# meco-group/omg-tools

Measured on AMD Instinct MI355X. Metric: MPC solves/sec, 1024-agent Holonomic Point2point batch per GPU, higher is better.
Workload: dtype f64

## Files before the change

### omg-tools_amd/csrc/omgx_core.h

```cpp
#pragma once
#include <stdint.h>
#include <math.h>

#ifdef OMGX_HOST_PORT
#define OMGX_FN inline
#define OMGX_HD inline
#define OMGX_HDF inline
#else
#define OMGX_FN __device__ __forceinline__
#define OMGX_HD __host__ __device__ inline
#define OMGX_HDF __host__ __device__ __forceinline__
#endif

#ifdef OMGX_HOST_PORT
#include <vector>
static thread_local std::vector<double> omgx_rbak;
#endif
#ifdef OMGX_COUNT_FACT
#include <atomic>
static std::atomic<long> omgx_dbg_nfact(0);
static std::atomic<long> omgx_dbg_cnt[12];
#endif
namespace omgx {

// ... 839 lines not shown
  const bool is_row = c.tid() < total_rows;
  const bool is_blk = wave >= row_waves && wave < row_waves + nm;
  int r = c.tid();
  BMat M = Ms[0];
  if (is_row) { int mi = 0; while (r >= Ms[mi].rows) { r -= Ms[mi].rows; ++mi; } M = Ms[mi]; }
  else if (is_blk) { M = Ms[wave - row_waves]; r = -1; }
  double* iv = (M.dinv >= 0) ? dinvb + M.dinv : colb + M.pan;
  double* gb = colb + M.pan + M.nfact;
  double* bb = gb + 16;
  const int br = baddr_k<KIND>(M, r > 0 ? r : 0, 0);
  int badl = 0;
  for (int jb = 0; jb < nmax; jb += OMGX_NB) {
    const bool live = (is_row || is_blk) && jb < M.nfact;
    const int nb = (M.nfact - jb) < OMGX_NB ? (M.nfact - jb) : OMGX_NB;
    const int q1 = nb > 1 ? 1 : 0, q2 = nb > 2 ? 2 : 0, q3 = nb > 3 ? 3 : 0;
    double v0 = 0.0, v1 = 0.0, v2 = 0.0, v3 = 0.0;
    if (live && is_blk) {
      const int a = lane & 15, kq = lane >> 4;
      const bool in_blk = a < nb;
      const int ra = baddr_k<KIND>(M, jb + (in_blk ? a : 0), 0);
      typedef double v4d __attribute__((ext_vector_type(4)));
      v4d acc = {0.0, 0.0, 0.0, 0.0}, acc2 = {0.0, 0.0, 0.0, 0.0};
      int k0 = 0;
      for (; k0 + 8 <= jb; k0 += 8) {
        const double u_a = A[ra + k0 + kq], t_a = iv[k0 + kq], u_b = A[ra + k0 + 4 + kq], t_b = iv[k0 + 4 + kq];
        const double ua = in_blk ? u_a : 0.0, ub = in_blk ? u_b : 0.0;
        acc = __builtin_amdgcn_mfma_f64_16x16x4f64(ua * t_a, ua, acc, 0, 0, 0);
        acc2 = __builtin_amdgcn_mfma_f64_16x16x4f64(ub * t_b, ub, acc2, 0, 0, 0);
      }
      for (; k0 < jb; k0 += 4) {
        const double u_a = A[ra + k0 + kq], t_a = iv[k0 + kq];
        const double ua = in_blk ? u_a : 0.0;
        acc = __builtin_amdgcn_mfma_f64_16x16x4f64(ua * t_a, ua, acc, 0, 0, 0);
      }
      acc += acc2;
      {
        const int gr = lane >> 4, gc = lane & 15;
        if (gc <= gr) {
          const bool ok = gr < nb && gc < nb;
          const double orig = A[baddr_k<KIND>(M, jb + (ok ? gr : 0), jb + (ok ? gc : 0))];
          gb[gr * 4 + gc] = ok ? orig - acc[0] : (gr == gc ? 1.0 : 0.0);
        }
      }
      c.wave_sync();
      const Blk4 B = blk4_from(gb[0], gb[4], gb[5], gb[8], gb[9], gb[10], gb[12], gb[13], gb[14], gb[15]);
      if (lane == 0) {
        bb[0] = B.l10; bb[1] = B.l20; bb[2] = B.l21; bb[3] = B.l30; bb[4] = B.l31; bb[5] = B.l32;
        bb[6] = B.d0; bb[7] = B.d1; bb[8] = B.d2; bb[9] = B.d3;
      }
      if (lane < nb) {
        const double dq = lane == 0 ? B.d0 : (lane == 1 ? B.d1 : (lane == 2 ? B.d2 : B.d3));
        const double iq = lane == 0 ? B.i0 : (lane == 1 ? B.i1 : (lane == 2 ? B.i2 : B.i3));
        const bool pos_ok = (jb + lane < M.npos) ? (dq > 0.0) : (dq < 0.0);
        if (!pos_ok) badl = 1;
        bb[10 + lane] = iq;
      }
    } else if (live && r >= jb + nb) {
      const int b0 = baddr_k<KIND>(M, jb, 0), b1 = baddr_k<KIND>(M, jb + q1, 0), b2 = baddr_k<KIND>(M, jb + q2, 0), b3 = baddr_k<KIND>(M, jb + q3, 0);
      v0 = A[br + jb]; v1 = A[br + jb + q1]; v2 = A[br + jb + q2]; v3 = A[br + jb + q3];
#pragma unroll 4
      for (int k = 0; k < jb; ++k) {
        const double tk = iv[k], ur = A[br + k];
        const double w = ur * tk;
        v0 -= w * A[b0 + k]; v1 -= w * A[b1 + k]; v2 -= w * A[b2 + k]; v3 -= w * A[b3 + k];
      }
    }
    c.sync();
    if (live && is_row && r >= jb) {
      const double l10 = bb[0], l20 = bb[1], l21 = bb[2], l30 = bb[3], l31 = bb[4], l32 = bb[5];
      const double d0 = bb[6], d1 = bb[7], d2 = bb[8], d3 = bb[9];
      if (r < jb + nb) {
        const int q = r - jb;
        iv[jb + q] = bb[10 + q];
        if (q == 1) { A[br + jb] = l10 * d0; }
        else if (q == 2) { A[br + jb] = l20 * d0; A[br + jb + 1] = l21 * d1; }
        else if (q == 3) { A[br + jb] = l30 * d0; A[br + jb + 1] = l31 * d1; A[br + jb + 2] = l32 * d2; }
        A[br + jb + q] = q == 0 ? d0 : (q == 1 ? d1 : (q == 2 ? d2 : d3));
      } else {
        const double u0 = v0;
        const double u1 = v1 - u0 * l10;
        const double u2 = v2 - u0 * l20 - u1 * l21;
        const double u3 = v3 - u0 * l30 - u1 * l31 - u2 * l32;
        A[br + jb] = u0;
        if (nb > 1) A[br + jb + 1] = u1;
        if (nb > 2) A[br + jb + 2] = u2;
        if (nb > 3) A[br + jb + 3] = u3;
      }
    }
    c.sync();
  }
  *bad = c.rmax(badl ? 1.0 : 0.0) > 0.0 ? 1 : 0;
}
#endif

template <int KIND, class C>
OMGX_FN void ldl_blocked(const C& c, const BMat* Ms, int nm, double* A, double* dinvb, double* colb, double* stage, int* bad) {
  int nmax = 0, total_rows = 0;
  for (int i = 0; i < nm; ++i) { if (Ms[i].nfact > nmax) nmax = Ms[i].nfact; total_rows += Ms[i].rows; }
  int badl = 0;
  int mi_own = 0, r_own = c.tid();
  BMat M_own = Ms[0];
  if (c.tid() < total_rows) {
    while (r_own >= Ms[mi_own].rows) { r_own -= Ms[mi_own].rows; ++mi_own; }
    M_own = Ms[mi_own];
  }
  OMGX_TIC();
  for (int jb = 0; jb < nmax; jb += OMGX_NB) {
    OMGX_PFOR(it, total_rows) {
      int mi = mi_own, r = r_own;
      BMat M = M_own;
      if (it != c.tid()) {
        mi = 0; r = it;
        while (r >= Ms[mi].rows) { r -= Ms[mi].rows; ++mi; }
        M = Ms[mi];
      }
      if (jb >= M.nfact || r < jb) continue;
      const int nb = (M.nfact - jb) < OMGX_NB ? (M.nfact - jb) : OMGX_NB;
      const Blk4 B = blk4_factor<KIND>(M, A, jb, nb);
      if (r < jb + nb) {
        const int q = r - jb;
        double* st = stage + mi * OMGX_STAGE_LD + q * 4;
        const double dq = q == 0 ? B.d0 : (q == 1 ? B.d1 : (q == 2 ? B.d2 : B.d3));
        const double iq = q == 0 ? B.i0 : (q == 1 ? B.i1 : (q == 2 ? B.i2 : B.i3));
        if (q == 1) { st[0] = B.l10; }
        else if (q == 2) { st[0] = B.l20; st[1] = B.l21; }
        else if (q == 3) { st[0] = B.l30; st[1] = B.l31; st[2] = B.l32; }
        st[q] = dq;
        const bool pos_ok = (jb + q < M.npos) ? (dq > 0.0) : (dq < 0.0);
        if (!pos_ok) badl = 1;
        if (M.dinv >= 0) dinvb[M.dinv + jb + q] = iq;
        stage[mi * OMGX_STAGE_LD + 16 + q] = iq;
        if (q == 0) for (int qq = nb; qq < OMGX_NB; ++qq) stage[mi * OMGX_STAGE_LD + 16 + qq] = 0.0;
        double* pr = colb + M.pan + r * OMGX_PAN_LD;
        pr[0] = 0.0; pr[1] = 0.0; pr[2] = 0.0; pr[3] = 0.0;
      } else {
        const int base = baddr_k<KIND>(M, r, jb);
        const double a0 = A[base];
        const double l1 = A[base + (nb > 1 ? 1 : 0)], l2 = A[base + (nb > 2 ? 2 : 0)], l3 = A[base + (nb > 3 ? 3 : 0)];
        const double a1 = nb > 1 ? l1 : 0.0;
        const double a2 = nb > 2 ? l2 : 0.0;
        const double a3 = nb > 3 ? l3 : 0.0;
        const double u0 = a0;
        const double u1 = a1 - u0 * B.l10;
        const double u2 = a2 - u0 * B.l20 - u1 * B.l21;
        const double u3 = a3 - u0 * B.l30 - u1 * B.l31 - u2 * B.l32;
        const double p0 = u0 * B.i0, p1 = nb > 1 ? u1 * B.i1 : 0.0, p2 = nb > 2 ? u2 * B.i2 : 0.0,
                     p3 = nb > 3 ? u3 * B.i3 : 0.0;
        double* pr = colb + M.pan + r * OMGX_PAN_LD;
        pr[0] = u0; pr[1] = nb > 1 ? u1 : 0.0; pr[2] = nb > 2 ? u2 : 0.0; pr[3] = nb > 3 ? u3 : 0.0;
        const bool fact_row = r < M.nfact;
        A[base] = fact_row ? p0 : u0;
        if (nb > 1) A[base + 1] = fact_row ? p1 : u1;
        if (nb > 2) A[base + 2] = fact_row ? p2 : u2;
        if (nb > 3) A[base + 3] = fact_row ? p3 : u3;
      }
    }
    c.sync();
    OMGX_TOC(PH_LA);
    OMGX_PFOR(it, nm * 16) {
      const int mi = it >> 4, q = (it >> 2) & 3, k = it & 3;
      const BMat M = Ms[mi];
      if (jb < M.nfact && jb + q < M.nfact && k <= q) A[baddr_k<KIND>(M, jb + q, jb + k)] = stage[mi * OMGX_STAGE_LD + (it & 15)];
    }
    OMGX_TOC(PH_LS);
    int tile0 = 0;
    for (int mi = 0; mi < nm; ++mi) {
      const BMat M = Ms[mi];
      const int s0 = jb + OMGX_NB;
      if (s0 >= M.nfact) continue;
      const int tr = (M.rows - s0 + 15) >> 4, tc = (M.nfact - s0 + 15) >> 4;
#ifdef OMGX_HOST_PORT
      (void)tile0; (void)tr; (void)tc;
      for (int r = s0; r < M.rows; ++r) {
        const int kmax = r < M.nfact ? r : M.nfact - 1;
        for (int k = s0; k <= kmax; ++k) {
          double acc = 0.0;
          for (int q = 0; q < OMGX_NB; ++q)
            acc += colb[M.pan + r * OMGX_PAN_LD + q] * (colb[M.pan + k * OMGX_PAN_LD + q] * stage[mi * OMGX_STAGE_LD + 16 + q]);
          A[baddr_k<KIND>(M, r, k)] -= acc;
        }
      }
#else
      const int lane = c.lane(), nwm = c.nwaves() - 1;
      for (int ti = (c.wave() - tile0) & nwm; ti < tr; ti += nwm + 1) {
        const int R0 = s0 + 16 * ti;
        for (int tj = 0; tj < tc; ++tj) {
          const int K0 = s0 + 16 * tj;
          if (K0 > R0 + 15 && R0 + 15 < M.nfact) break;
          const int ra = R0 + (lane & 15), kb = K0 + (lane & 15), q = lane >> 4;
          const double av_l = colb[M.pan + (ra < M.rows ? ra : M.rows - 1) * OMGX_PAN_LD + q];
          const double bv_l = colb[M.pan + (kb < M.nfact ? kb : M.nfact - 1) * OMGX_PAN_LD + q];
          const double iv_l = stage[mi * OMGX_STAGE_LD + 16 + q];
          typedef double v4d __attribute__((ext_vector_type(4)));
          v4d acc;
          const int col = K0 + (lane & 15);
          int ad[4]; bool ok[4];
#pragma unroll
          for (int i = 0; i < 4; ++i) {
            const int row = R0 + (lane >> 4) + 4 * i;
            ok[i] = row < M.rows && col < M.nfact && (row >= M.nfact || col <= row);
            ad[i] = ok[i] ? baddr_k<KIND>(M, row, col) : M.a;
          }
          double al[4];
#pragma unroll
          for (int i = 0; i < 4; ++i) al[i] = A[ad[i]];
#pragma unroll
          for (int i = 0; i < 4; ++i) acc[i] = ok[i] ? al[i] : 0.0;
          const double av = (ra < M.rows) ? -av_l : 0.0;
          const double bv = (kb < M.nfact) ? bv_l * iv_l : 0.0;
          acc = __builtin_amdgcn_mfma_f64_16x16x4f64(av, bv, acc, 0, 0, 0);
#pragma unroll
          for (int i = 0; i < 4; ++i) if (ok[i]) A[ad[i]] = acc[i];
        }
      }
      tile0 += tr;
#endif
    }
    c.sync();
    OMGX_TOC(PH_LB);
  }
  *bad = c.rmax(badl ? 1.0 : 0.0) > 0.0 ? 1 : 0;
}

template <bool WAVE_ONLY, bool HBM, bool ROOT_LDS>
OMGX_HDF void kkt_describe_fill(const Dims& d, const Kkt& K, BMat* Ms) {
  const int pan0 = (OMGX_BMAT_DOUBLES + OMGX_STAGE_LD) * (OMGX_MAX_LEAF + 1);
  int pan = pan0;
  for (int l = 0; l < d.n_leaf; ++l) {
    BMat& M = Ms[l];
    if constexpr (WAVE_ONLY) {
      M.a = K.d_off[l]; M.ld = K.ld(l); M.nfact = K.nl(l); M.rows = K.nl(l) + K.nc(l) + 1; M.npos = M.nfact;
      M.dinv = K.leaf_off[l]; M.pan = K.lf_w[l]; M.cpl = K.cpl_ptr[l]; M.bw = K.lf_kind[l] ? -1 : K.lf_band[l]; M.pad_ = K.lf_ldb[l];
      continue;
    }
    M.a = K.d_off[l]; M.ld = K.ld(l); M.nfact = K.nl(l); M.rows = K.nl(l) + K.nc(l) + 1; M.npos = M.nfact;
    M.dinv = K.leaf_off[l]; M.pan = pan; pan += HBM ? OMGX_PAN_SMALL(M.nfact) : OMGX_PAN_LD * M.rows; M.cpl = K.cpl_ptr[l]; M.bw = K.leaf_bw[l];
  }
  BMat& Mr = Ms[d.n_leaf];
  Mr.a = ROOT_LDS ? 0 : K.d_off[d.n_leaf]; Mr.ld = 0; Mr.nfact = d.nr; Mr.rows = d.nr + 1; Mr.npos = d.n_root; Mr.dinv = -1; Mr.pan = pan0; Mr.cpl = 0; Mr.bw = d.nr;
  Mr.pad_ = K.d_off[d.n_leaf];
}

template <class C>
OMGX_FN void kkt_describe(const C& c, const Dims& d, const Kkt& K, Work& w, bool sync_after = true) {
  const int who = c.nthr() > 64 ? 64 : 0;
  if (c.tid() == who) kkt_describe_fill<C::wave_only, C::hbm, C::root_lds>(d, K, (BMat*)w.col);
  if (sync_after) c.sync();
}

template <class C>
OMGX_FN void kkt_descriptors(const C& c, const Dims& d, const Tables& T, Work& w, bool sync_after = true) {
  if constexpr (C::wave_only) {
    const int t0 = c.nthr() > 64 ? 64 : 0, nt = c.nthr() > 64 ? 64 : c.nthr();
    const int i0 = c.tid() - t0, n = (d.n_leaf + 1) * (int)(sizeof(BMat) / sizeof(int32_t));
    int32_t* Ms = (int32_t*)w.col;
    if (i0 >= 0 && i0 < nt) for (int i = i0; i < n; i += nt) Ms[i] = T.bmat_img[i];
    if (sync_after) c.sync();
  } else {
    Kkt K; K.bind(d, T, w.kkt);
    kkt_describe(c, d, K, w, sync_after);
  }
}

#ifndef OMGX_HOST_PORT
OMGX_FN WPanel wpanel_leaf(const BMat& M) {
  WPanel P; P.base = M.a; P.ld = M.ld; P.n = M.nfact; P.nreg = M.rows - 2; P.nvec = 2; P.npos = M.nfact; P.bw = M.bw;
  P.vrow = M.rows - 2; P.band = M.bw; P.ldb = M.pad_; P.wbase = M.pan;
  return P;
}
OMGX_FN WPanel wpanel_root(const BMat& M, int n_root) {
  WPanel P; P.base = M.a; P.ld = 0; P.n = M.nfact; P.nreg = M.nfact; P.nvec = 1; P.npos = n_root; P.bw = M.nfact;
  P.vrow = M.nfact; P.band = -1; P.ldb = 0; P.wbase = 0;
  return P;
}

struct DiagLeaf { int base, n, S, dinv, dl; };
OMGX_FN DiagLeaf diag_leaf(const BMat& M) {
  DiagLeaf L;
  L.base = __builtin_amdgcn_readfirstlane(M.a); L.n = __builtin_amdgcn_readfirstlane(M.nfact);
  L.S = __builtin_amdgcn_readfirstlane(M.pan); L.dinv = __builtin_amdgcn_readfirstlane(M.dinv); L.dl = 4 * L.dinv;
  return L;
}

template <class C>
OMGX_FN int kkt_factor_wave(const C& c, const Dims& d, const Kkt& K, Work& w) {
  typedef double v4d __attribute__((ext_vector_type(4)));
  const BMat* Ms = (const BMat*)w.col;
  const int lane = c.lane(), wave = c.wave(), nw = c.nwaves();
  const int koff = (int)(w.kkt - omgx_lds);
  OMGX_TIC();
  int badl = 0;
#ifdef OMGX_PROFILE
  const long long tw0_ = clock64();
#endif
  for (int l = wave; l < d.n_leaf; l += nw) {
    const int kind_bw = __builtin_amdgcn_readfirstlane(Ms[l].bw);
    if (kind_bw < 0) {
      const DiagLeaf L = diag_leaf(Ms[l]);
      const double dj = w.kkt[L.base + (lane < L.n ? lane : 0)];
      if (lane < L.n) { w.dinv[L.dinv + lane] = rcp_pivot(dj); if (!(dj > 0.0)) badl = 1; }
      continue;
    }
    const WPanel P = wpanel_leaf(Ms[l]);
    badl |= (kind_bw <= 8) ? wave_ldl<OMGX_WAVE_COLS, 8, true>(koff, P) : wave_ldl<OMGX_WAVE_COLS, OMGX_WAVE_COLS, true>(koff, P);
    wave_fence();
    const double dl = wave_dinv<true>(w.kkt, P);
    if (lane < P.n) w.dinv[Ms[l].dinv + lane] = dl;
  }
#ifdef OMGX_PROFILE
  if (c.tid() == 0) { c.prof[PH_F_SCALE] += clock64() - tw0_; c.prof[PH_F_PARK] += 1; }
#endif
  if (c.rmax(badl ? 1.0 : 0.0) > 0.0) return 1;
  OMGX_TOC(PH_F_LEAF);
  double* R = K.R();
  for (int base = 0; base < d.n_leaf; base += nw) {
    const int l = base + wave;
    v4d acc00 = {0.0, 0.0, 0.0, 0.0}, acc10 = acc00, acc11 = acc00;
    int nc1 = 0, ci_b0 = 0, ci_b1 = 0, ci_a[8];
    bool sparse = false;
#pragma unroll
    for (int i = 0; i < 8; ++i) ci_a[i] = 0;
    if (l < d.n_leaf) {
      const BMat M = Ms[l];
      sparse = __builtin_amdgcn_readfirstlane(M.bw) < 0;
      if (!sparse) {
      const int n = __builtin_amdgcn_readfirstlane(M.nfact), ld = __builtin_amdgcn_readfirstlane(M.ld);
      nc1 = __builtin_amdgcn_readfirstlane(M.rows) - n;
      const double* Wt = w.kkt + __builtin_amdgcn_readfirstlane(M.pan);
      const double* di = w.dinv + __builtin_amdgcn_readfirstlane(M.dinv);
      const int32_t* ci = K.cpl_idx + __builtin_amdgcn_readfirstlane(M.cpl);
      const int cb0 = lane & 15, cb1 = 16 + (lane & 15);
      ci_b0 = ci[cb0 < nc1 - 1 ? cb0 : 0]; ci_b1 = ci[cb1 < nc1 - 1 ? cb1 : 0];
#pragma unroll
      for (int i = 0; i < 8; ++i) {
        const int ca = 16 * (i >> 2) + (lane >> 4) + 4 * (i & 3);
        ci_a[i] = ca < nc1 - 1 ? ci[ca] : d.nr;
      }
      const int r0 = lane & 15, r1 = 16 + (lane & 15), q = lane >> 4;
      const int r0c = r0 < nc1 ? r0 : nc1 - 1, r1c = r1 < nc1 ? r1 : nc1 - 1;
      const bool two = nc1 > 16;
      for (int j0 = 0; j0 < n; j0 += 4) {
        const int j = j0 + q, jc = j < n ? j : n - 1;
        const double w0 = Wt[r0c * ld + jc], w1 = Wt[r1c * ld + jc], dj = di[jc];
        const double b0 = (r0 < nc1 && j < n) ? w0 : 0.0, b1 = (r1 < nc1 && j < n) ? w1 : 0.0;
        acc00 = __builtin_amdgcn_mfma_f64_16x16x4f64(b0 * dj, b0, acc00, 0, 0, 0);
        if (two) {
          acc10 = __builtin_amdgcn_mfma_f64_16x16x4f64(b1 * dj, b0, acc10, 0, 0, 0);
          acc11 = __builtin_amdgcn_mfma_f64_16x16x4f64(b1 * dj, b1, acc11, 0, 0, 0);
        }
      }
      }
    }
    const int lend = base + nw < d.n_leaf ? base + nw : d.n_leaf;
    for (int lr = base; lr < lend; ++lr) {
      if (l == lr && !sparse) {
        const int cb0 = lane & 15, cb1 = 16 + (lane & 15);
#pragma unroll
        for (int i = 0; i < 4; ++i) {
          const int ca0 = (lane >> 4) + 4 * i, ca1 = 16 + ca0;
          if (ca0 < nc1 && cb0 < nc1 - 1 && cb0 <= ca0) R[tri(ci_a[i], ci_b0)] -= acc00[i];
          if (ca1 < nc1 && cb0 < nc1 - 1) R[tri(ci_a[4 + i], ci_b0)] -= acc10[i];
          if (ca1 < nc1 && cb1 < nc1 - 1 && cb1 <= ca1) R[tri(ci_a[4 + i], ci_b1)] -= acc11[i];
        }
      } else if (l == lr) {
        const DiagLeaf L = diag_leaf(Ms[l]);
        const int j = lane < L.n ? lane : 0;
        const bool on = lane < L.n;
        const double* A = w.kkt + L.base + j;
        const double di = w.dinv[L.dinv + j];
        const double vt = A[(1 + L.S) * L.n], rj = A[(2 + L.S) * L.n];
        const int pt = d.n_root - 1;
        double vs[4]; int ps[4];
#pragma unroll
        for (int s = 0; s < 4; ++s) {
          const bool has = s < L.S;
          ps[s] = has ? K.dl_pos[L.dl + s * L.n + j] : -1;
          const double v = A[(1 + (has ? s : 0)) * L.n];
          vs[s] = (has && on && ps[s] >= 0) ? v : 0.0;
        }
        if (on) {
#pragma unroll
          for (int s = 0; s < 4; ++s) {
            if (ps[s] < 0 || s >= L.S) continue;
            const double u = vs[s] * di;
#pragma unroll
            for (int s2 = 0; s2 <= s; ++s2) {
              if (ps[s2] < 0) continue;
              const int pa = ps[s] > ps[s2] ? ps[s] : ps[s2], pb = ps[s] > ps[s2] ? ps[s2] : ps[s];
              R[tri(pa, pb)] -= u * vs[s2];
            }
            R[tri(pt, ps[s])] -= u * vt;
            R[tri(d.nr, ps[s])] -= u * rj;
          }
        }
        const double stt = c.wave_sum(on ? vt * di * vt : 0.0), srt = c.wave_sum(on ? rj * di * vt : 0.0);
        if (lane == 0) { R[tri(pt, pt)] -= stt; R[tri(d.nr, pt)] -= srt; }
      }
      c.sync();
    }
  }
  OMGX_TOC(PH_F_SCHUR);
  int badr = 0;
  if (wave == 0) {
    const WPanel P = wpanel_root(Ms[d.n_leaf], d.n_root);
#ifdef OMGX_PROFILE
    const long long tr0_ = clock64();
#endif
    badr = wave_ldl<OMGX_WAVE_COLS, OMGX_WAVE_COLS, false>(koff, P);
#ifdef OMGX_PROFILE
    if (c.tid() == 0) c.prof[PH_F_SWEEP] += clock64() - tr0_;
#endif
  }
  const int bad = c.rmax(badr ? 1.0 : 0.0) > 0.0 ? 2 : 0;
  OMGX_TOC(PH_F_ROOT);
  return bad;
}

template <class C>
OMGX_FN int kkt_refactor_root_wave(const C& c, const Dims& d, const Kkt& K, Work& w) {
  const BMat* Ms = (const BMat*)w.col;
  const int koff = (int)(w.kkt - omgx_lds);
  OMGX_TIC();
  int badr = 0;
  if (c.wave() == 0) badr = wave_ldl<OMGX_WAVE_COLS, OMGX_WAVE_COLS, false>(koff, wpanel_root(Ms[d.n_leaf], d.n_root));
  const int bad = c.rmax(badr ? 1.0 : 0.0) > 0.0 ? 2 : 0;
  OMGX_TOC(PH_F_ROOT);
  return bad;
}

template <class C>
OMGX_FN void kkt_solve_wave(const C& c, const Dims& d, const Kkt& K, Work& w, double* sol) {
  const BMat* Ms = (const BMat*)w.col;
  const int lane = c.lane(), wave = c.wave(), nw = c.nwaves();
  const int koff = (int)(w.kkt - omgx_lds);
  OMGX_TIC();
  if (wave == 0) {
    const WPanel P = wpanel_root(Ms[d.n_leaf], d.n_root);
    const double dl = wave_dinv<false>(w.kkt, P);
    const double y = w.kkt[wcarried<false>(P, P.n) + (lane < P.n ? lane : 0)];
    const double x = wave_bwd<OMGX_WAVE_COLS, false>(koff, P, dl, y * dl);
    if (lane < P.n) sol[d.root_off + lane] = x;
  }
  c.sync();
  OMGX_TOC(PH_K_ROOT);
  double* xg = w.col + OMGX_BMAT_DOUBLES * (OMGX_MAX_LEAF + 1) + wave * 64;
  for (int l = wave; l < d.n_leaf; l += nw) {
    const BMat M = Ms[l];
    if (__builtin_amdgcn_readfirstlane(M.bw) < 0) {
      const DiagLeaf L = diag_leaf(M);
      const int j = lane < L.n ? lane : 0;
      const double* A = w.kkt + L.base + j;
      double acc = A[(2 + L.S) * L.n] - A[(1 + L.S) * L.n] * sol[d.root_off + d.n_root - 1];
      for (int s = 0; s < L.S; ++s) {
        const int ps = K.dl_pos[L.dl + s * L.n + j];
        acc = fma(-A[(1 + s) * L.n], sol[d.root_off + (ps < 0 ? 0 : ps)] * (ps < 0 ? 0.0 : 1.0), acc);
      }
      if (lane < L.n) sol[L.dinv + lane] = acc * w.dinv[L.dinv + j];
      continue;
    }
    const WPanel P = wpanel_uniform(wpanel_leaf(M));
    const int n = P.n, nc = P.nreg + 1 - P.n, ld = P.ld;
    const int32_t* ci = K.cpl_idx + __builtin_amdgcn_readfirstlane(M.cpl);
    if (lane < nc) xg[lane] = sol[d.root_off + ci[lane]];
    wave_fence();
    const int j = lane < n ? lane : 0;
    const double* Wt = w.kkt + P.wbase + j;
    double acc = Wt[nc * ld];
#pragma unroll 4
    for (int a = 0; a < nc; ++a) acc = fma(-Wt[a * ld], xg[a], acc);
    const int dv = __builtin_amdgcn_readfirstlane(M.dinv);
    const double dl = w.dinv[dv + j];
    const double x = wave_bwd<OMGX_WAVE_COLS, true>(koff, P, dl, acc * dl);
    if (lane < n) sol[dv + lane] = x;
    wave_fence();
  }
  c.sync();
  OMGX_TOC(PH_K_BWD);
}

template <class C>
OMGX_FN void kkt_solve2_wave(const C& c, const Dims& d, const Kkt& K, Work& w, double* out, bool with_y = false) {
  const BMat* Ms = (const BMat*)w.col;
  const int lane = c.lane(), wave = c.wave(), nw = c.nwaves();
  const int koff = (int)(w.kkt - omgx_lds);
  double* xg0 = w.col + OMGX_BMAT_DOUBLES * (OMGX_MAX_LEAF + 1);
  double* R = K.R();
  const int rrow = tri(d.nr, 0);
  for (int base = 0; base < d.n_leaf; base += nw) {
    const int l = base + wave;
    double* xg = xg0 + wave * 64;
    if (l < d.n_leaf && __builtin_amdgcn_readfirstlane(Ms[l].bw) >= 0) {
      const BMat M = Ms[l];
      const WPanel P = wpanel_uniform(wpanel_leaf(M));
      const int n = P.n, nc = P.nreg + 1 - P.n, ld = P.ld;
      const int j = lane < n ? lane : 0;
      double* Wt = w.kkt + P.wbase;
      const int dv = __builtin_amdgcn_readfirstlane(M.dinv);
      const double dl = w.dinv[dv + j];
      const double y = wave_fwd_r<true>(koff, P, dl, Wt[nc * ld + j]);
      if (lane < n) { Wt[nc * ld + lane] = y; xg[lane] = y * dl; }
      wave_fence();
      const int a = lane < nc ? lane : 0;
      double acc = 0.0;
#pragma unroll 4
      for (int q = 0; q < n; ++q) acc = fma(Wt[a * ld + q], xg[q], acc);
      wave_fence();
      if (lane < nc) xg[lane] = acc;
    }
    c.sync();
    if (wave == 0) {
      const int lend = base + nw < d.n_leaf ? base + nw : d.n_leaf;
      for (int lr = base; lr < lend; ++lr) {
        const BMat M = Ms[lr];
        if (__builtin_amdgcn_readfirstlane(M.bw) >= 0) {
          const int nc = __builtin_amdgcn_readfirstlane(M.rows) - 1 - __builtin_amdgcn_readfirstlane(M.nfact);
          const int32_t* ci = K.cpl_idx + __builtin_amdgcn_readfirstlane(M.cpl);
          const double* xs = xg0 + (lr - base) * 64;
          if (lane < nc) R[rrow + ci[lane]] -= xs[lane];
        } else {
          const DiagLeaf L = diag_leaf(M);
          const int j = lane < L.n ? lane : 0;
          const bool on = lane < L.n;
          const double* A = w.kkt + L.base + j;
          const double u = A[(2 + L.S) * L.n] * w.dinv[L.dinv + j];
          for (int s = 0; s < L.S; ++s) {
            const int ps = K.dl_pos[L.dl + s * L.n + j];
            if (on && ps >= 0) R[rrow + ps] -= A[(1 + s) * L.n] * u;
          }
          const double st = c.wave_sum(on ? A[(1 + L.S) * L.n] * u : 0.0);
          if (lane == 0) R[rrow + d.n_root - 1] -= st;
        }
        wave_fence();
      }
    }
    c.sync();
  }
  if (wave == 0) {
    const WPanel P = wpanel_root(Ms[d.n_leaf], d.n_root);
    const double dl = wave_dinv<false>(w.kkt, P);
    const int j = lane < P.n ? lane : 0;
    const double y = wave_fwd_r<false>(koff, P, dl, w.kkt[wcarried<false>(P, P.n) + j]);
    const double x = wave_bwd_r<false>(koff, P, dl, y * dl);
    if (lane < (with_y ? P.n : d.n_root)) out[d.root_off + lane] = x;
  }
  c.sync();
  double* xg = xg0 + wave * 64;
  for (int l = wave; l < d.n_leaf; l += nw) {
    const BMat M = Ms[l];
    if (__builtin_amdgcn_readfirstlane(M.bw) < 0) {
      const DiagLeaf L = diag_leaf(M);
      const int j = lane < L.n ? lane : 0;
      const double* A = w.kkt + L.base + j;
      double acc = A[(2 + L.S) * L.n] - A[(1 + L.S) * L.n] * out[d.root_off + d.n_root - 1];
      for (int s = 0; s < L.S; ++s) {
        const int ps = K.dl_pos[L.dl + s * L.n + j];
        acc = fma(-A[(1 + s) * L.n], out[d.root_off + (ps < 0 ? 0 : ps)] * (ps < 0 ? 0.0 : 1.0), acc);
      }
      if (lane < L.n) out[L.dinv + lane] = acc * w.dinv[L.dinv + j];
      continue;
    }
    const WPanel P = wpanel_uniform(wpanel_leaf(M));
    const int n = P.n, nc = P.nreg + 1 - P.n, ld = P.ld;
    const int32_t* ci = K.cpl_idx + __builtin_amdgcn_readfirstlane(M.cpl);
    if (lane < nc) xg[lane] = out[d.root_off + ci[lane]];
    wave_fence();
    const int j = lane < n ? lane : 0;
    const double* Wt = w.kkt + P.wbase + j;
    double acc = Wt[nc * ld];
#pragma unroll 4
    for (int a = 0; a < nc; ++a) acc = fma(-Wt[a * ld], xg[a], acc);
    const int dv = __builtin_amdgcn_readfirstlane(M.dinv);
    const double dl = w.dinv[dv + j];
    const double x = wave_bwd_r<true>(koff, P, dl, acc * dl);
    if (lane < n) out[dv + lane] = x;
    wave_fence();
  }
  c.sync();
}
#endif

template <class C>
OMGX_FN int kkt_factor(const C& c, const Dims& d, const Kkt& K, Work& w) {
#ifndef OMGX_HOST_PORT
  if constexpr (C::wave_only) return kkt_factor_wave(c, d, K, w);
#endif
  if constexpr (C::wave_only) return 1; else {
  int bad = 0;
  OMGX_TIC();
  BMat* Ms = (BMat*)w.col;
  double* stage = w.col + OMGX_BMAT_DOUBLES * (OMGX_MAX_LEAF + 1);
  if (d.n_leaf > 0) {
#ifdef OMGX_HOST_PORT
    ldl_left4(c, Ms, d.n_leaf, w.kkt, w.dinv, w.col, &bad);
#else
    {
      int total_rows = 0, nmax = 0; bool room = true;
      for (int l = 0; l < d.n_leaf; ++l) {
        total_rows += Ms[l].rows; if (Ms[l].nfact > nmax) nmax = Ms[l].nfact;
        if (Ms[l].nfact + 30 > OMGX_PAN_LD * Ms[l].rows) room = false;
      }
      const bool coop = room && ((total_rows + 63) >> 6) + d.n_leaf <= c.nwaves();
      if constexpr (C::hbm) ldl_left4(c, Ms, d.n_leaf, w.kkt, w.dinv, w.col, &bad);
      else if (coop) ldl_left4_coop<1>(c, Ms, d.n_leaf, w.kkt, w.dinv, w.col, &bad, total_rows, nmax);
      else ldl_left4(c, Ms, d.n_leaf, w.kkt, w.dinv, w.col, &bad);
    }
#endif
#ifdef OMGX_COUNT_FACT
    if (bad) ++omgx_dbg_cnt[0];
#endif
    if (bad) return 1;
  }
  OMGX_TOC(PH_F_LEAF);
  if constexpr (C::root_lds) {
    const double* Rg = K.R();
    const int nrd = ((d.nr + 1) * (d.nr + 2)) / 2;
    OMGX_PFOR(i, nrd) w.root[i] = Rg[i];
    c.sync();
  }
  double* R = C::root_lds ? w.root : K.R();
#ifdef OMGX_HOST_PORT
  for (int l = 0; l < d.n_leaf; ++l) {
    const int n = K.nl(l), nc = K.nc(l), ld = K.ld(l);
    const double* Wt = K.P(l) + n * ld;
    const double* di = w.dinv + K.leaf_off[l];
    const int32_t* ci = K.cpl_idx + K.cpl_ptr[l];
    for (int ai = 0; ai <= nc; ++ai) for (int ak = 0; ak <= ai && ak < nc; ++ak) {
      double acc = 0.0;
      for (int j = 0; j < n; ++j) acc += Wt[ai * ld + j] * Wt[ak * ld + j] * di[j];
      R[tri(ai < nc ? ci[ai] : d.nr, ci[ak])] -= acc;
    }
  }
#else
  {
    const int lane = c.lane();
    for (int l = 0; l < d.n_leaf; ++l) {
      const BMat M = Ms[l];
      const int n = M.nfact, nc = M.rows - M.nfact;
      OMGX_PANEL_STRIDES(C, M, sr, sc);
      const double* Wt = w.kkt + M.a + n * sr;
      const double* di = w.dinv + M.dinv;
      const int32_t* ci = K.cpl_idx + M.cpl;
      const int tn = (nc + 15) >> 4, nwm = c.nwaves() - 1;
      int tile = 0;
      for (int ti = 0; ti < tn; ++ti) for (int tj = 0; tj <= ti; ++tj, ++tile) {
        if ((tile & nwm) != c.wave()) continue;
        typedef double v4d __attribute__((ext_vector_type(4)));
        v4d acc = {0.0, 0.0, 0.0, 0.0};
        const int ra = 16 * ti + (lane & 15), rb = 16 * tj + (lane & 15), q = lane >> 4;
        const int rac = ra < nc ? ra : nc - 1, rbc = rb < nc ? rb : nc - 1;
        const double* Wa = Wt + rac * sr;
        const double* Wb = Wt + rbc * sr;
        for (int j0 = 0; j0 < n; j0 += 32) {
          double wa[8], wb[8], wd[8];
#pragma unroll
          for (int u = 0; u < 8; ++u) {
            const int j = j0 + 4 * u + q;
            const int jc = j < n ? j : n - 1;
            wa[u] = Wa[jc * sc]; wd[u] = di[jc]; wb[u] = Wb[jc * sc];
          }
#pragma unroll
          for (int u = 0; u < 8; ++u) {
            const int j = j0 + 4 * u + q;
            const double av = (ra < nc && j < n) ? wa[u] * wd[u] : 0.0;
            const double bv = (rb < nc && j < n) ? wb[u] : 0.0;
            acc = __builtin_amdgcn_mfma_f64_16x16x4f64(av, bv, acc, 0, 0, 0);
          }
        }
        const int cb = 16 * tj + (lane & 15);
        for (int i = 0; i < 4; ++i) {
          const int ca = 16 * ti + (lane >> 4) + 4 * i;
          if (ca < nc && cb < nc - 1 && cb <= ca) R[tri(ca < nc - 1 ? ci[ca] : d.nr, ci[cb])] -= acc[i];
        }
      }
      c.sync();
    }
  }
#endif
  c.sync();
  OMGX_TOC(PH_F_SCHUR);
#ifdef OMGX_HOST_PORT
  if (d.wave_ok) omgx_rbak.assign(R, R + ((size_t)(d.nr + 1) * (d.nr + 2)) / 2);
#endif
  ldl_blocked<2>(c, Ms + d.n_leaf, 1, C::root_lds ? w.root : w.kkt, w.dinv, w.col, stage, &bad);
  OMGX_TOC(PH_F_ROOT);
#ifdef OMGX_COUNT_FACT
  if (bad) ++omgx_dbg_cnt[1];
#endif
  return bad ? 2 : 0;
  }
}

template <class C>
OMGX_FN void kkt_root_before_retry(const C& c, const Dims& d, const Kkt& K, Work& w) {
#ifdef OMGX_HOST_PORT
  double* R = K.R();
  for (size_t i = 0; i < omgx_rbak.size(); ++i) R[i] = omgx_rbak[i];
#endif
}
template <class C>
OMGX_FN int kkt_refactor_root(const C& c, const Dims& d, const Kkt& K, Work& w) {
#ifndef OMGX_HOST_PORT
  if constexpr (!C::wave_only) return 1;
  else return kkt_refactor_root_wave(c, d, K, w);
#else
  int bad = 0;
  BMat* Ms = (BMat*)w.col;
  double* stage = w.col + OMGX_BMAT_DOUBLES * (OMGX_MAX_LEAF + 1);
  double* R = K.R();
  omgx_rbak.assign(R, R + ((size_t)(d.nr + 1) * (d.nr + 2)) / 2);
  ldl_blocked<2>(c, Ms + d.n_leaf, 1, w.kkt, w.dinv, w.col, stage, &bad);
  return bad ? 2 : 0;
#endif
}

template <class C, class Addr>
OMGX_FN void trsv_bwd4(const C& c, const double* A, Addr L, int n, double* y, const double* iv = nullptr) {
  const int lane = c.lane(), nln = c.nlanes();
  const int nblk = (n + 3) >> 2;
  for (int bk = nblk - 1; bk >= 0; --bk) {
    const int jb = 4 * bk;
    const int nb = (n - jb) < 4 ? (n - jb) : 4;
    const int q1 = nb > 1 ? 1 : 0, q2 = nb > 2 ? 2 : 0, q3 = nb > 3 ? 3 : 0;
    const double m1 = nb > 1 ? 1.0 : 0.0, m2 = nb > 2 ? 1.0 : 0.0, m3 = nb > 3 ? 1.0 : 0.0;
    const double r0 = y[jb], r1 = m1 * y[jb + q1], r2 = m2 * y[jb + q2], r3 = m3 * y[jb + q3];
    const double s0 = iv ? iv[jb] : 1.0, s1 = iv ? iv[jb + q1] : 1.0, s2 = iv ? iv[jb + q2] : 1.0;
    const double l10 = m1 * A[L(jb + q1, jb)] * s0;
    const double l20 = m2 * A[L(jb + q2, jb)] * s0, l21 = m2 * A[L(jb + q2, jb + (q2 ? 1 : 0))] * s1;
    const double l30 = m3 * A[L(jb + q3, jb)] * s0, l31 = m3 * A[L(jb + q3, jb + (q3 ? 1 : 0))] * s1,
                 l32 = m3 * A[L(jb + q3, jb + (q3 ? 2 : 0))] * s2;
    const double x3 = r3, x2 = r2 - l32 * x3, x1 = r1 - l21 * x2 - l31 * x3, x0 = r0 - l10 * x1 - l20 * x2 - l30 * x3;
    for (int i = lane; i < jb + nb; i += nln) {
      if (i < jb) {
        const double si = iv ? iv[i] : 1.0;
        y[i] -= si * (A[L(jb, i)] * x0 + m1 * A[L(jb + q1, i)] * x1 + m2 * A[L(jb + q2, i)] * x2 + m3 * A[L(jb + q3, i)] * x3);
      } else {
        const int q = i - jb;
        y[i] = q == 0 ? x0 : (q == 1 ? x1 : (q == 2 ? x2 : x3));
      }
    }
    c.wave_sync();
  }
}

template <class C, class Addr>
OMGX_FN void trsv_fwd4(const C& c, const double* A, Addr L, int n, double* y, const double* iv = nullptr) {
  const int lane = c.lane(), nln = c.nlanes();
  const int nblk = (n + 3) >> 2;
  for (int bk = 0; bk < nblk; ++bk) {
    const int jb = 4 * bk;
    const int nb = (n - jb) < 4 ? (n - jb) : 4;
    const int q1 = nb > 1 ? 1 : 0, q2 = nb > 2 ? 2 : 0, q3 = nb > 3 ? 3 : 0;
    const double m1 = nb > 1 ? 1.0 : 0.0, m2 = nb > 2 ? 1.0 : 0.0, m3 = nb > 3 ? 1.0 : 0.0;
    const double s0 = iv ? iv[jb] : 1.0, s1 = iv ? iv[jb + q1] : 1.0, s2 = iv ? iv[jb + q2] : 1.0, s3 = iv ? iv[jb + q3] : 1.0;
    const double l10 = m1 * A[L(jb + q1, jb)] * s0;
    const double l20 = m2 * A[L(jb + q2, jb)] * s0, l21 = m2 * A[L(jb + q2, jb + (q2 ? 1 : 0))] * s1;
    const double l30 = m3 * A[L(jb + q3, jb)] * s0, l31 = m3 * A[L(jb + q3, jb + (q3 ? 1 : 0))] * s1,
                 l32 = m3 * A[L(jb + q3, jb + (q3 ? 2 : 0))] * s2;
    const double x0 = y[jb], x1 = m1 * (y[jb + q1] - l10 * x0), x2 = m2 * (y[jb + q2] - l20 * x0 - l21 * x1),
                 x3 = m3 * (y[jb + q3] - l30 * x0 - l31 * x1 - l32 * x2);
    c.wave_sync();
    for (int i = jb + lane; i < n; i += nln) {
      if (i >= jb + nb) {
        y[i] -= A[L(i, jb)] * s0 * x0 + m1 * A[L(i, jb + q1)] * s1 * x1 + m2 * A[L(i, jb + q2)] * s2 * x2 + m3 * A[L(i, jb + q3)] * s3 * x3;
      } else {
        const int q = i - jb;
        y[i] = q == 0 ? x0 : (q == 1 ? x1 : (q == 2 ? x2 : x3));
      }
    }
    c.wave_sync();
  }
}

template <class C>
OMGX_FN void kkt_solve(const C& c, const Dims& d, const Kkt& K, Work& w, double* sol) {
#ifndef OMGX_HOST_PORT
// ... 1113 lines not shown
```

### omg-tools_amd/csrc/omgx_wave.h

```cpp
#pragma once

namespace omgx {

__device__ __forceinline__ double readlane_d(double v, int lane) {
  const int lo = __builtin_amdgcn_readlane(__double2loint(v), lane);
  const int hi = __builtin_amdgcn_readlane(__double2hiint(v), lane);
  return __hiloint2double(hi, lo);
}

__device__ __forceinline__ void wave_fence() {
  __builtin_amdgcn_fence(__ATOMIC_RELEASE, "wavefront");
  __builtin_amdgcn_wave_barrier();
  __builtin_amdgcn_fence(__ATOMIC_ACQUIRE, "wavefront");
}

struct WPanel { int base, ld, n, nreg, nvec, npos, bw, vrow, band, ldb, wbase; };

__device__ __forceinline__ WPanel wpanel_uniform(const WPanel& Q) {
  WPanel P;
  P.base = __builtin_amdgcn_readfirstlane(Q.base); P.ld = __builtin_amdgcn_readfirstlane(Q.ld);
  P.n = __builtin_amdgcn_readfirstlane(Q.n);
  P.nreg = __builtin_amdgcn_readfirstlane(Q.nreg); P.nvec = __builtin_amdgcn_readfirstlane(Q.nvec);
  P.npos = __builtin_amdgcn_readfirstlane(Q.npos); P.bw = __builtin_amdgcn_readfirstlane(Q.bw);
  P.vrow = __builtin_amdgcn_readfirstlane(Q.vrow); P.band = __builtin_amdgcn_readfirstlane(Q.band);
  P.ldb = __builtin_amdgcn_readfirstlane(Q.ldb); P.wbase = __builtin_amdgcn_readfirstlane(Q.wbase);
  return P;
}

template <bool BANDED>
__device__ __forceinline__ int wcarried(const WPanel& P, int r) {
  return BANDED ? P.wbase + (r - P.n) * P.ld : P.base + ((r * (r + 1)) >> 1);
}
template <bool BANDED>
__device__ __forceinline__ int wsym(const WPanel& P, int i) {
  return BANDED ? P.base + i * P.ldb + P.band - i : P.base + ((i * (i + 1)) >> 1);
}

extern __shared__ double omgx_lds[];

template <int NC, int BW, bool BANDED>
__device__ __forceinline__ int wave_ldl(int off, const WPanel Pin) {
  const double* A = omgx_lds + off;
  double* Aw = omgx_lds + off;
  const WPanel P = wpanel_uniform(Pin);
  const int lane = threadIdx.x & 63;
  const int n = P.n;
  const bool has_row = lane < P.nreg;
  const bool sym_row = lane < n;
  const int rl = has_row ? lane : 0;
  const int ra = rl < n ? wsym<BANDED>(P, rl) : wcarried<BANDED>(P, rl);
  const int klo = (BANDED && rl < n && rl > P.band) ? rl - P.band : 0;
  const int khi = rl < n ? rl : n - 1;
  double a[NC];
#pragma unroll
  for (int k = 0; k < NC; ++k) {
    const int kk = k < klo ? klo : (k > khi ? khi : k);
    const double v = A[ra + kk];
    a[k] = (has_row && k >= klo && k <= khi) ? v : 0.0;
  }
  const int v0a = wcarried<BANDED>(P, P.vrow), v1a = wcarried<BANDED>(P, P.vrow + (P.nvec > 1 ? 1 : 0));
  double yv0, yv1;
  {
    const int c = sym_row ? lane : 0;
    const double v0 = A[v0a + c], v1 = A[v1a + c];
    yv0 = (P.nvec > 0 && sym_row) ? v0 : 0.0;
    yv1 = (P.nvec > 1 && sym_row) ? v1 : 0.0;
  }
  int bad = 0;
#pragma unroll
  for (int j = 0; j < NC; ++j) {
    const double dj = readlane_d(a[j], j);
    const bool okp = (j < P.npos) ? (dj > 0.0) : (dj < 0.0);
    bad |= (j < n && !okp) ? 1 : 0;
    const double inv = rcp_pivot(dj);
    const double li = a[j] * inv;
    {
      int ln = lane;
      asm volatile("" : "+v"(ln));
      const double lm = ln > j ? li : 0.0;
      const double y0j = readlane_d(yv0, j), y1j = readlane_d(yv1, j);
      yv0 = fma(-lm, j < n ? y0j : 0.0, yv0);
      yv1 = fma(-lm, j < n ? y1j : 0.0, yv1);
    }
#pragma unroll
    for (int c = j / 4; c < NC / 4; ++c) {
      if (4 * c > j + BW) continue;
      double s[4];
#pragma unroll
      for (int q = 0; q < 4; ++q) s[q] = readlane_d(a[j], 4 * c + q);
#pragma unroll
      for (int q = 0; q < 4; ++q) {
        const int k = 4 * c + q;
        if (k > j && k <= j + BW) a[k] = fma(-li, s[q], a[k]);
      }
      asm volatile("" : "+v"(a[4 * c]), "+v"(a[4 * c + 1]), "+v"(a[4 * c + 2]), "+v"(a[4 * c + 3]));
    }
  }
  if (!bad) {
    if (has_row) {
#pragma unroll
      for (int k = 0; k < NC; ++k) {
        int ln = lane;
        asm volatile("" : "+v"(ln));
        if (k < n && (sym_row ? (k <= ln && k >= klo) : true)) Aw[ra + k] = a[k];
      }
    }
    if (sym_row) {
      if (P.nvec > 0) Aw[v0a + lane] = yv0;
      if (P.nvec > 1) Aw[v1a + lane] = yv1;
    }
  }
  return bad;
}

template <int NC, int W>
__device__ __forceinline__ int root_ldl_4w_wave(int off, const WPanel P, int xoff) {
  constexpr int NL = NC / 4;
  constexpr int BS = 72;
  constexpr bool act = W < 4;
  const double* A = omgx_lds + off;
  double* Aw = omgx_lds + off;
  double* X = omgx_lds + xoff;
  const int lane = threadIdx.x & 63;
  const int n = P.n;
  const bool has_row = lane < n;
  const int rl = has_row ? lane : 0;
  const int ra = wsym<false>(P, rl);
  double a[NL];
#pragma unroll
  for (int c = 0; c < NL; ++c) {
    const int j = 4 * c + (act ? W : 0);
    const int jj = j > rl ? rl : j;
    const double v = A[ra + jj];
    a[c] = (has_row && j <= rl) ? v : 0.0;
  }
  const int v0a = wcarried<false>(P, P.vrow);
  double yv0;
  {
    const double v0 = A[v0a + rl];
    yv0 = (P.nvec > 0 && has_row) ? v0 : 0.0;
  }
  int bad = 0;
  if (W == 0) {
    X[lane] = a[0];
    const double d0 = readlane_d(a[0], 0);
    if (lane == 0) X[64] = rcp_pivot(d0);
  }
  __syncthreads();
#pragma unroll
  for (int k = 0; k < NC; ++k) {
    if (k < n) {
      const double* buf = X + (k & 1) * BS;
      double* nxt = X + ((k + 1) & 1) * BS;
      if (act) {
        const bool pub = (k + 1 < NC) && (((k + 1) & 3) == W);
        const int c1 = pub ? (k + 1) >> 2 : 0;
        const double colk = buf[lane], inv = buf[64], s1 = buf[pub ? k + 1 : 0], dk = buf[k];
        const double li = colk * inv;
        if (pub) {
          a[c1] = fma(-li, s1, a[c1]);
          nxt[lane] = a[c1];
          const double d1 = readlane_d(a[c1], k + 1);
          if (lane == 0) nxt[64] = rcp_pivot(d1);
        }
        const bool okp = (k < P.npos) ? (dk > 0.0) : (dk < 0.0);
        bad |= okp ? 0 : 1;
        {
          int ln = lane;
          asm volatile("" : "+v"(ln));
          const double lm = ln > k ? li : 0.0;
          const double y0k = readlane_d(yv0, k);
          yv0 = fma(-lm, y0k, yv0);
        }
#pragma unroll
        for (int c = k >> 2; c < NL; ++c) {
          const int j = 4 * c + W;
          if (j > k + 1) {
            const double s = buf[j];
            a[c] = fma(-li, s, a[c]);
          }
        }
      }
      __syncthreads();
    }
  }
  if (!bad && act) {
    if (has_row) {
#pragma unroll
      for (int c = 0; c < NL; ++c) {
        const int j = 4 * c + W;
        if (j < n && j <= lane) Aw[ra + j] = a[c];
      }
    }
    if (W == 0 && has_row && P.nvec > 0) Aw[v0a + lane] = yv0;
  }
  if (W == 0 && lane == 0) X[2 * BS] = bad ? 1.0 : 0.0;
  __syncthreads();
  const int bad_all = X[2 * BS] != 0.0 ? 1 : 0;
  __syncthreads();
  return bad_all;
}

template <int NC>
__device__ __forceinline__ int root_ldl_4w(int off, const WPanel Pin, int xoff) {
  static_assert(NC % 4 == 0, "columns are dealt to four waves");
  const WPanel P = wpanel_uniform(Pin);
  const int wv = __builtin_amdgcn_readfirstlane((int)(threadIdx.x >> 6));
  switch (wv) {
    case 0: return root_ldl_4w_wave<NC, 0>(off, P, xoff);
    case 1: return root_ldl_4w_wave<NC, 1>(off, P, xoff);
    case 2: return root_ldl_4w_wave<NC, 2>(off, P, xoff);
    case 3: return root_ldl_4w_wave<NC, 3>(off, P, xoff);
    default: return root_ldl_4w_wave<NC, 4>(off, P, xoff);
  }
}

template <bool BANDED>
__device__ __forceinline__ double wave_dinv(const double* A, const WPanel P) {
  const int lane = threadIdx.x & 63;
  const int c = lane < P.n ? lane : 0;
  const double d = A[wsym<BANDED>(P, c) + c];
  return lane < P.n ? rcp_pivot(d) : 0.0;
}

template <int NC, bool BANDED>
__device__ __forceinline__ double wave_bwd(int off, const WPanel Pin, double dinvl, double z) {
  const double* A = omgx_lds + off;
  const WPanel P = wpanel_uniform(Pin);
  const int lane = threadIdx.x & 63;
  const int n = P.n;
  double lt[NC];
  const int c = lane < n ? lane : 0;
#pragma unroll
  for (int i = 0; i < NC; ++i) {
    const int ic = i < n ? i : n - 1;
    const bool in = !BANDED || ic - c <= P.band;
    const int cc = in ? c : ic - P.band;
    const double v = A[wsym<BANDED>(P, ic) + cc];
    lt[i] = (i < n && lane < i && in) ? v * dinvl : 0.0;
  }
  double x = lane < n ? z : 0.0;
#pragma unroll
  for (int i = NC - 1; i >= 1; --i) {
    if (i < n) x = fma(-lt[i], readlane_d(x, i), x);
  }
  return x;
}

template <bool BANDED>
__device__ __forceinline__ double wave_fwd_r(int off, const WPanel Pin, double dinvl, double r) {
  const double* A = omgx_lds + off;
  const WPanel P = wpanel_uniform(Pin);
  const int lane = threadIdx.x & 63;
  const int n = P.n;
  const int rl = lane < n ? lane : 0;
  const int ra = wsym<BANDED>(P, rl);
  const int klo = (BANDED && rl > P.band) ? rl - P.band : 0;
  double y = lane < n ? r : 0.0;
  for (int j0 = 0; j0 < n; j0 += 8) {
    double l[8];
#pragma unroll
    for (int q = 0; q < 8; ++q) {
      const int j = j0 + q;
      const int kk = j < klo ? klo : (j > rl ? rl : j);
      const double v = A[ra + kk];
      const double dk = readlane_d(dinvl, j);
      l[q] = (lane < n && j >= klo && j < rl) ? v * dk : 0.0;
    }
#pragma unroll
    for (int q = 0; q < 8; ++q) {
      const int j = j0 + q;
      const double yj = readlane_d(y, j);
      y = fma(-l[q], j < n ? yj : 0.0, y);
    }
  }
  return y;
}

template <bool BANDED>
__device__ __forceinline__ double wave_bwd_r(int off, const WPanel Pin, double dinvl, double z) {
  const double* A = omgx_lds + off;
  const WPanel P = wpanel_uniform(Pin);
  const int lane = threadIdx.x & 63;
  const int n = P.n;
  const int c = lane < n ? lane : 0;
  double x = lane < n ? z : 0.0;
  for (int i0 = ((n + 7) & ~7) - 8; i0 >= 0; i0 -= 8) {
    double l[8];
#pragma unroll
    for (int q = 0; q < 8; ++q) {
      const int i = i0 + q;
      const int ic = i < n ? i : n - 1;
      const bool in = !BANDED || ic - c <= P.band;
      const int cc = in ? c : ic - P.band;
      const double v = A[wsym<BANDED>(P, ic) + cc];
      l[q] = (i < n && lane < i && in) ? v * dinvl : 0.0;
    }
#pragma unroll
    for (int q = 7; q >= 0; --q) {
      const int i = i0 + q;
      const double xi = readlane_d(x, i);
      x = fma(-l[q], i < n ? xi : 0.0, x);
    }
  }
  return x;
}

}
```

Before: 3.551 million.

## Specialize leaf LDL for small panels and streamline pivot sign checks

```diff
diff --git a/omg-tools_amd/csrc/omgx_core.h b/omg-tools_amd/csrc/omgx_core.h
--- a/omg-tools_amd/csrc/omgx_core.h
+++ b/omg-tools_amd/csrc/omgx_core.h
@@ -1165,7 +1165,9 @@
       continue;
     }
     const WPanel P = wpanel_leaf(Ms[l]);
-    badl |= (kind_bw <= 8) ? wave_ldl<OMGX_WAVE_COLS, 8, true>(koff, P) : wave_ldl<OMGX_WAVE_COLS, OMGX_WAVE_COLS, true>(koff, P);
+    const int leaf_n = __builtin_amdgcn_readfirstlane(Ms[l].nfact);
+    if (wave_leaf_small(leaf_n, kind_bw)) badl |= wave_ldl<OMGX_LEAF_COLS_SMALL, OMGX_LEAF_BW_SMALL, true, 2>(koff, P);
+    else badl |= (kind_bw <= 8) ? wave_ldl<OMGX_WAVE_COLS, 8, true, 2>(koff, P) : wave_ldl<OMGX_WAVE_COLS, OMGX_WAVE_COLS, true, 2>(koff, P);
     wave_fence();
     const double dl = wave_dinv<true>(w.kkt, P);
     if (lane < P.n) w.dinv[Ms[l].dinv + lane] = dl;
@@ -1269,7 +1271,7 @@
 #ifdef OMGX_PROFILE
     const long long tr0_ = clock64();
 #endif
-    badr = wave_ldl<OMGX_WAVE_COLS, OMGX_WAVE_COLS, false>(koff, P);
+    badr = wave_ldl<OMGX_WAVE_COLS, OMGX_WAVE_COLS, false, 1>(koff, P);
 #ifdef OMGX_PROFILE
     if (c.tid() == 0) c.prof[PH_F_SWEEP] += clock64() - tr0_;
 #endif
@@ -1285,7 +1287,7 @@
   const int koff = (int)(w.kkt - omgx_lds);
   OMGX_TIC();
   int badr = 0;
-  if (c.wave() == 0) badr = wave_ldl<OMGX_WAVE_COLS, OMGX_WAVE_COLS, false>(koff, wpanel_root(Ms[d.n_leaf], d.n_root));
+  if (c.wave() == 0) badr = wave_ldl<OMGX_WAVE_COLS, OMGX_WAVE_COLS, false, 1>(koff, wpanel_root(Ms[d.n_leaf], d.n_root));
   const int bad = c.rmax(badr ? 1.0 : 0.0) > 0.0 ? 2 : 0;
   OMGX_TOC(PH_F_ROOT);
   return bad;
@@ -1333,7 +1335,8 @@
     for (int a = 0; a < nc; ++a) acc = fma(-Wt[a * ld], xg[a], acc);
     const int dv = __builtin_amdgcn_readfirstlane(M.dinv);
     const double dl = w.dinv[dv + j];
-    const double x = wave_bwd<OMGX_WAVE_COLS, true>(koff, P, dl, acc * dl);
+    const double x = wave_leaf_small(n, P.bw) ? wave_bwd<OMGX_LEAF_COLS_SMALL, true>(koff, P, dl, acc * dl)
+                                              : wave_bwd<OMGX_WAVE_COLS, true>(koff, P, dl, acc * dl);
     if (lane < n) sol[dv + lane] = x;
     wave_fence();
   }
diff --git a/omg-tools_amd/csrc/omgx_wave.h b/omg-tools_amd/csrc/omgx_wave.h
--- a/omg-tools_amd/csrc/omgx_wave.h
+++ b/omg-tools_amd/csrc/omgx_wave.h
@@ -12,6 +12,26 @@
   __builtin_amdgcn_fence(__ATOMIC_RELEASE, "wavefront");
   __builtin_amdgcn_wave_barrier();
   __builtin_amdgcn_fence(__ATOMIC_ACQUIRE, "wavefront");
+}
+
+__host__ __device__ __forceinline__ unsigned pivot_wrong_sign(unsigned bad, int hi, int lo, int j, int npos, int n) {
+  const unsigned flip = (unsigned)(npos - 1 - j) & 0x80000000u;
+  const unsigned lim = j < n ? 0x7fefffffu : 0xffffffffu;
+#if defined(__HIP_DEVICE_COMPILE__)
+  unsigned w, t;
+  const unsigned flip_s = __builtin_amdgcn_readfirstlane(flip), lim_s = __builtin_amdgcn_readfirstlane(lim);
+  asm("s_min_u32 %2, %4, 1\n\t"
+      "s_xor_b32 %1, %3, %5\n\t"
+      "s_or_b32 %1, %1, %2\n\t"
+      "s_add_u32 %1, %1, -1\n\t"
+      "s_cmp_gt_u32 %1, %6\n\t"
+      "s_cselect_b32 %0, 1, %0"
+      : "+s"(bad), "=&s"(w), "=&s"(t) : "s"(hi), "s"(lo), "s"(flip_s), "s"(lim_s) : "scc");
+  return bad;
+#else
+  const unsigned k = ((unsigned)hi ^ flip) | (lo != 0 ? 1u : 0u);
+  return (k - 1u > lim) ? 1u : bad;
+#endif
 }
 
 struct WPanel { int base, ld, n, nreg, nvec, npos, bw, vrow, band, ldb, wbase; };
@@ -27,6 +47,10 @@
   return P;
 }
 
+#define OMGX_LEAF_COLS_SMALL 36
+#define OMGX_LEAF_BW_SMALL   5
+__host__ __device__ __forceinline__ bool wave_leaf_small(int n, int bw) { return n <= OMGX_LEAF_COLS_SMALL && bw <= OMGX_LEAF_BW_SMALL; }
+
 template <bool BANDED>
 __device__ __forceinline__ int wcarried(const WPanel& P, int r) {
   return BANDED ? P.wbase + (r - P.n) * P.ld : P.base + ((r * (r + 1)) >> 1);
@@ -38,8 +62,9 @@
 
 extern __shared__ double omgx_lds[];
 
-template <int NC, int BW, bool BANDED>
+template <int NC, int BW, bool BANDED, int NVEC>
 __device__ __forceinline__ int wave_ldl(int off, const WPanel Pin) {
+  static_assert(NC % 4 == 0 && NVEC >= 1 && NVEC <= 2, "columns go in chunks of four; one or two vector rows");
   const double* A = omgx_lds + off;
   double* Aw = omgx_lds + off;
   const WPanel P = wpanel_uniform(Pin);
@@ -58,29 +83,35 @@
     const double v = A[ra + kk];
     a[k] = (has_row && k >= klo && k <= khi) ? v : 0.0;
   }
-  const int v0a = wcarried<BANDED>(P, P.vrow), v1a = wcarried<BANDED>(P, P.vrow + (P.nvec > 1 ? 1 : 0));
-  double yv0, yv1;
+  const int v0a = wcarried<BANDED>(P, P.vrow), v1a = wcarried<BANDED>(P, P.vrow + (NVEC > 1 && P.nvec > 1 ? 1 : 0));
+  double yv0, yv1 = 0.0;
   {
     const int c = sym_row ? lane : 0;
-    const double v0 = A[v0a + c], v1 = A[v1a + c];
+    const double v0 = A[v0a + c];
     yv0 = (P.nvec > 0 && sym_row) ? v0 : 0.0;
-    yv1 = (P.nvec > 1 && sym_row) ? v1 : 0.0;
-  }
-  int bad = 0;
+    if (NVEC > 1) {
+      const double v1 = A[v1a + c];
+      yv1 = (P.nvec > 1 && sym_row) ? v1 : 0.0;
+    }
+  }
+  unsigned bad = 0;
 #pragma unroll
   for (int j = 0; j < NC; ++j) {
-    const double dj = readlane_d(a[j], j);
-    const bool okp = (j < P.npos) ? (dj > 0.0) : (dj < 0.0);
-    bad |= (j < n && !okp) ? 1 : 0;
+    const int dlo = __builtin_amdgcn_readlane(__double2loint(a[j]), j), dhi = __builtin_amdgcn_readlane(__double2hiint(a[j]), j);
+    const double dj = __hiloint2double(dhi, dlo);
+    bad = pivot_wrong_sign(bad, dhi, dlo, j, P.npos, n);
     const double inv = rcp_pivot(dj);
     const double li = a[j] * inv;
     {
       int ln = lane;
       asm volatile("" : "+v"(ln));
       const double lm = ln > j ? li : 0.0;
-      const double y0j = readlane_d(yv0, j), y1j = readlane_d(yv1, j);
+      const double y0j = readlane_d(yv0, j);
       yv0 = fma(-lm, j < n ? y0j : 0.0, yv0);
-      yv1 = fma(-lm, j < n ? y1j : 0.0, yv1);
+      if (NVEC > 1) {
+        const double y1j = readlane_d(yv1, j);
+        yv1 = fma(-lm, j < n ? y1j : 0.0, yv1);
+      }
     }
 #pragma unroll
     for (int c = j / 4; c < NC / 4; ++c) {
@@ -102,15 +133,16 @@
       for (int k = 0; k < NC; ++k) {
         int ln = lane;
         asm volatile("" : "+v"(ln));
-        if (k < n && (sym_row ? (k <= ln && k >= klo) : true)) Aw[ra + k] = a[k];
+        const int kh = sym_row ? ln : khi;
+        if (k >= klo && k <= kh) Aw[ra + k] = a[k];
       }
     }
     if (sym_row) {
       if (P.nvec > 0) Aw[v0a + lane] = yv0;
-      if (P.nvec > 1) Aw[v1a + lane] = yv1;
-    }
-  }
-  return bad;
+      if (NVEC > 1 && P.nvec > 1) Aw[v1a + lane] = yv1;
+    }
+  }
+  return (int)bad;
 }
 
 template <int NC, int W>
```

After: 3.613 million, median of 6. 1.8% higher.
